# facebookresearch/jepa

Measured on AMD Instinct MI355X. Metric: V-JEPA pretrain clips/sec (fwd+bwd+EMA), higher is better.
Workload: dtype bf16; 1 GPU; V-JEPA pretrain step ViT-L/16 16x224x224, B=24/GPU, 2 multiblock masks (vitl16.yaml); global_batch=24, per_gpu_batch=24, parallelism=dp1, hw_queues=4

## Files before the change

### jepa_amd/csrc/common.hpp

```cpp
#pragma once
#include <hip/hip_runtime.h>
#include <stdint.h>
#include <stdio.h>

typedef uint16_t bf16_t;

typedef __attribute__((ext_vector_type(8))) __bf16 bf16x8_t;
typedef __attribute__((ext_vector_type(4))) float f32x4_t;
typedef __attribute__((ext_vector_type(4))) uint32_t u32x4_t;
typedef __attribute__((ext_vector_type(2))) uint32_t u32x2_t;

#define VJ_WAVE 64

__device__ __forceinline__ float bf2f(bf16_t v) { return __uint_as_float(((uint32_t)v) << 16); }

__device__ __forceinline__ bf16_t f2bf(float f) {
  uint32_t u = __float_as_uint(f);
  if ((u & 0x7fffffffu) > 0x7f800000u) return (bf16_t)((u >> 16) | 0x40u);
  u += 0x7fffu + ((u >> 16) & 1u);
  return (bf16_t)(u >> 16);
}
__device__ __forceinline__ uint32_t pack_bf2(float lo, float hi) {
  typedef __bf16 bf2_t __attribute__((ext_vector_type(2)));
  bf2_t v = {(__bf16)lo, (__bf16)hi};
  return __builtin_bit_cast(uint32_t, v);
}
__device__ __forceinline__ uint32_t pack_bf2_opaque(float lo, float hi) {
  uint32_t w = pack_bf2(lo, hi);
  asm("" : "+v"(w));
  return w;
}
__device__ __forceinline__ float bf_lo(uint32_t w) { return __uint_as_float(w << 16); }
__device__ __forceinline__ float bf_hi(uint32_t w) { return __uint_as_float(w & 0xffff0000u); }

__device__ __forceinline__ float wave_sum(float v) {
#pragma unroll
  for (int o = 32; o > 0; o >>= 1) v += __shfl_xor(v, o, 64);
  return v;
}
__device__ __forceinline__ float row16_sum(float v) {
  v += __int_as_float(__builtin_amdgcn_update_dpp(0, __float_as_int(v), 0x128, 0xf, 0xf, false));
  v += __int_as_float(__builtin_amdgcn_update_dpp(0, __float_as_int(v), 0x124, 0xf, 0xf, false));
  v += __int_as_float(__builtin_amdgcn_update_dpp(0, __float_as_int(v), 0x122, 0xf, 0xf, false));
  v += __int_as_float(__builtin_amdgcn_update_dpp(0, __float_as_int(v), 0x121, 0xf, 0xf, false));
  return v;
}
template <int N>
__device__ __forceinline__ void block4_stage(float (*red)[4], const float (&v)[N]) {
  float w[N];
#pragma unroll
  for (int k = 0; k < N; k++) w[k] = wave_sum(v[k]);
  if ((threadIdx.x & 63) == 0) {
#pragma unroll
    for (int k = 0; k < N; k++) red[k][threadIdx.x >> 6] = w[k];
  }
  __syncthreads();
}
__device__ __forceinline__ float block4_total(const float* red) { return red[0] + red[1] + red[2] + red[3]; }
__device__ __forceinline__ float wave_max(float v) {
#pragma unroll
  for (int o = 32; o > 0; o >>= 1) v = fmaxf(v, __shfl_xor(v, o, 64));
  return v;
}

typedef float f32x2_t __attribute__((ext_vector_type(2)));
__device__ __forceinline__ float twice_relu(float x) {
  float s;
  asm("v_add_f32 %0, %1, |%1|" : "=v"(s) : "v"(x));
  return s;
}
__device__ __forceinline__ f32x2_t half_erfc2_lp(f32x2_t x, f32x2_t& a) {
  a = (f32x2_t){__builtin_amdgcn_fmed3f(__builtin_fabsf(x[0]), 0.0f, 5.0f), __builtin_amdgcn_fmed3f(__builtin_fabsf(x[1]), 0.0f, 5.0f)};
  const f32x2_t c6 = {2.945814386e-05f, 2.945814386e-05f}, c5 = {-7.087827263e-04f, -7.087827263e-04f},
                 c4 = {7.746013931e-03f, 7.746013931e-03f}, c3 = {-5.260629358e-02f, -5.260629358e-02f},
                 c2 = {-4.596254594e-01f, -4.596254594e-01f}, c1 = {-1.150867238e+00f, -1.150867238e+00f},
                 c0 = {-1.000017643e+00f, -1.000017643e+00f};
  f32x2_t p = __builtin_elementwise_fma(c6, a, c5);
  p = __builtin_elementwise_fma(p, a, c4);
  p = __builtin_elementwise_fma(p, a, c3);
  p = __builtin_elementwise_fma(p, a, c2);
  p = __builtin_elementwise_fma(p, a, c1);
  p = __builtin_elementwise_fma(p, a, c0);
  return (f32x2_t){__builtin_amdgcn_exp2f(p[0]), __builtin_amdgcn_exp2f(p[1])};
}
__device__ __forceinline__ f32x2_t gelu2_lp(f32x2_t x) {
  f32x2_t a;
  const f32x2_t q = half_erfc2_lp(x, a);
  const f32x2_t s = {twice_relu(x[0]), twice_relu(x[1])};
  const f32x2_t half = {0.5f, 0.5f};
  return __builtin_elementwise_fma(s, half, -(a * q));
}
__device__ __forceinline__ void gelu_dgelu2_lp(f32x2_t x, f32x2_t& y, f32x2_t& d) {
  f32x2_t a;
  const f32x2_t q = half_erfc2_lp(x, a);
  const f32x2_t s = {twice_relu(x[0]), twice_relu(x[1])};
  const f32x2_t half = {0.5f, 0.5f};
  y = __builtin_elementwise_fma(s, half, -(a * q));
  const f32x2_t c = {-0.72134752044448170f, -0.72134752044448170f};
  const f32x2_t e = (x * c) * x;
  const f32x2_t g = {__builtin_amdgcn_exp2f(e[0]), __builtin_amdgcn_exp2f(e[1])};
  const f32x2_t hq = half - q;
  const f32x2_t phi = half + (f32x2_t){copysignf(hq[0], x[0]), copysignf(hq[1], x[1])};
  const f32x2_t k = {0.3989422804014327f, 0.3989422804014327f};
  d = __builtin_elementwise_fma(x * k, g, phi);
}

__device__ __forceinline__ int xcd_logical(int bid, int nblk) {
  const int qx = nblk >> 3, rx = nblk & 7, xcd = bid & 7, pos = bid >> 3;
  return (xcd < rx ? xcd * (qx + 1) : rx * (qx + 1) + (xcd - rx) * qx) + pos;
}

#include <atomic>
#define VJ_MAX_DEVICES 64
inline int vj_device_slot() {
  int dev = 0;
  if (hipGetDevice(&dev) != hipSuccess || dev < 0) dev = 0;
  return dev % VJ_MAX_DEVICES;
}
struct VjPerDeviceOnce {
  std::atomic<unsigned long long> done{0};
  template <class F>
  void operator()(F&& f) {
    const unsigned long long bit = 1ull << vj_device_slot();
    if (!(done.load(std::memory_order_acquire) & bit)) {
      f();
      done.fetch_or(bit, std::memory_order_release);
    }
  }
};

extern "C" const char* vj_last_error(void);
void vj_set_error(const char* fmt, ...);

#define VJ_CHECK_ARG(cond, ...)            \
  do {                                     \
    if (!(cond)) {                         \
      vj_set_error(__VA_ARGS__);           \
      return -1;                           \
    }                                      \
  } while (0)

#define VJ_LAUNCH_CHECK(name)                                              \
  do {                                                                     \
    hipError_t _e = hipGetLastError();                                     \
    if (_e != hipSuccess) {                                                \
      vj_set_error("%s: launch failed: %s", name, hipGetErrorString(_e)); \
      return (int)_e;                                                      \
    }                                                                      \
  } while (0)

__host__ __device__ static inline int64_t cdiv64(int64_t a, int64_t b) { return (a + b - 1) / b; }

static inline int rows_grid(int64_t rows, int64_t cap_blocks = 256 * 16) {
  int64_t g = cdiv64(rows, 4);
  if (g > cap_blocks) g = cap_blocks;
  if (g < 1) g = 1;
  return (int)g;
}
static inline int flat_grid(int64_t total, int64_t cap_blocks) {
  int64_t g = cdiv64(total, 256);
  if (g > cap_blocks) g = cap_blocks;
  return (int)g;
}
__device__ __forceinline__ int wave_lane() { return threadIdx.x & 63; }
__device__ __forceinline__ int64_t wave_row() { return (int64_t)blockIdx.x * 4 + (threadIdx.x >> 6); }
__device__ __forceinline__ int64_t wave_row_step() { return (int64_t)gridDim.x * 4; }

__device__ __forceinline__ void unpack8(const u32x4_t& w, float* v) {
#pragma unroll
  for (int i = 0; i < 4; i++) {
    v[2 * i] = bf_lo(w[i]);
    v[2 * i + 1] = bf_hi(w[i]);
  }
}
__device__ __forceinline__ void load8(const bf16_t* p, float* v) { unpack8(*(const u32x4_t*)p, v); }
__device__ __forceinline__ void store8(bf16_t* p, const float* v) {
  u32x4_t w;
#pragma unroll
  for (int i = 0; i < 4; i++) w[i] = pack_bf2(v[2 * i], v[2 * i + 1]);
  *(u32x4_t*)p = w;
}
__device__ __forceinline__ u32x2_t pack4_bf16(float a, float b, float c, float d) {
  u32x2_t w;
  w[0] = pack_bf2(a, b);
  w[1] = pack_bf2(c, d);
  return w;
}
__device__ __forceinline__ u32x4_t pack8_bf16(float4 lo, float4 hi) {
  u32x4_t o;
  o[0] = pack_bf2(lo.x, lo.y);
  o[1] = pack_bf2(lo.z, lo.w);
  o[2] = pack_bf2(hi.x, hi.y);
  o[3] = pack_bf2(hi.z, hi.w);
  return o;
}
__device__ __forceinline__ u32x4_t add_pos8(u32x4_t v, const float* pos) {
  const float4 p0 = *(const float4*)pos;
  const float4 p1 = *(const float4*)(pos + 4);
  v[0] = pack_bf2(bf_lo(v[0]) + p0.x, bf_hi(v[0]) + p0.y);
  v[1] = pack_bf2(bf_lo(v[1]) + p0.z, bf_hi(v[1]) + p0.w);
  v[2] = pack_bf2(bf_lo(v[2]) + p1.x, bf_hi(v[2]) + p1.y);
  v[3] = pack_bf2(bf_lo(v[3]) + p1.z, bf_hi(v[3]) + p1.w);
  return v;
}
```

### jepa_amd/csrc/layernorm.hip

```cpp
#include "common.hpp"
#include "options.hpp"
#include "internal.hpp"

#define LN_MAX_CHUNKS 4

static int ln_check_D(const char* who, int64_t D, bool rule = false) {
  VJ_CHECK_ARG(D % 8 == 0 && D <= 512 * LN_MAX_CHUNKS, rule ? "%s: D=%ld unsupported (need D%%8==0, D<=%d)" : "%s: D=%ld unsupported", who,
               (long)D, 512 * LN_MAX_CHUNKS);
  return 0;
}
static inline int ln_grid(int64_t rows) { return rows_grid(rows, 256 * 8); }

template <bool LOAD>
__device__ __forceinline__ float ln_row_mean(const bf16_t* xp, float (&v)[LN_MAX_CHUNKS][8], int lane, int D, float invD) {
  float s = 0.f;
#pragma unroll
  for (int i = 0; i < LN_MAX_CHUNKS; i++) {
    const int c = lane * 8 + i * 512;
    if (c < D) {
      if constexpr (LOAD) load8(xp + c, v[i]);
#pragma unroll
      for (int j = 0; j < 8; j++) s += v[i][j];
    }
  }
  return wave_sum(s) * invD;
}
__device__ __forceinline__ float ln_row_rstd(const float (&v)[LN_MAX_CHUNKS][8], float mean, int lane, int D, float invD, float eps) {
  float q = 0.f;
#pragma unroll
  for (int i = 0; i < LN_MAX_CHUNKS; i++) {
    if (lane * 8 + i * 512 < D) {
#pragma unroll
      for (int j = 0; j < 8; j++) {
        const float d = v[i][j] - mean;
        q += d * d;
      }
    }
  }
  return rsqrtf(wave_sum(q) * invD + eps);
}

__global__ __launch_bounds__(256) void layernorm_fwd_kernel(const bf16_t* __restrict__ x,
                                                            const float* __restrict__ gamma,
                                                            const float* __restrict__ beta, bf16_t* __restrict__ y,
                                                            float* __restrict__ mean_out, float* __restrict__ rstd_out,
                                                            int64_t rows, int D, float eps) {
  __shared__ __attribute__((aligned(16))) float4 gbs[LN_MAX_CHUNKS][4][64];
  const int lane = threadIdx.x & 63;
  for (int q = threadIdx.x; q < LN_MAX_CHUNKS * 64; q += 256) {
    const int i = q >> 6, l = q & 63, c = l * 8 + i * 512;
    if (c < D) {
      gbs[i][0][l] = *(const float4*)(gamma + c);
      gbs[i][1][l] = *(const float4*)(gamma + c + 4);
      gbs[i][2][l] = *(const float4*)(beta + c);
      gbs[i][3][l] = *(const float4*)(beta + c + 4);
    }
  }
  __syncthreads();
  const int64_t wave = (int64_t)blockIdx.x * 4 + (threadIdx.x >> 6);
  const int64_t nw = (int64_t)gridDim.x * 4;
  const float invD = 1.0f / (float)D;
  for (int64_t r = wave; r < rows; r += nw) {
    const bf16_t* xp = x + r * D;
    float v[LN_MAX_CHUNKS][8];
    const float mean = ln_row_mean<true>(xp, v, lane, D, invD);
    const float rstd = ln_row_rstd(v, mean, lane, D, invD, eps);
    bf16_t* yp = y + r * D;
#pragma unroll
    for (int i = 0; i < LN_MAX_CHUNKS; i++) {
      const int c = lane * 8 + i * 512;
      if (c < D) {
        const float4 g0 = gbs[i][0][lane], g1 = gbs[i][1][lane], b0 = gbs[i][2][lane], b1 = gbs[i][3][lane];
        const float gm[8] = {g0.x, g0.y, g0.z, g0.w, g1.x, g1.y, g1.z, g1.w};
        const float bt[8] = {b0.x, b0.y, b0.z, b0.w, b1.x, b1.y, b1.z, b1.w};
        float o[8];
#pragma unroll
        for (int j = 0; j < 8; j++) o[j] = (v[i][j] - mean) * rstd * gm[j] + bt[j];
        store8(yp + c, o);
      }
    }
    if (lane == 0 && mean_out) {
      mean_out[r] = mean;
      rstd_out[r] = rstd;
    }
  }
}

extern "C" int vj_layernorm_fwd(const void* x_bf16, const float* gamma, const float* beta, void* y_bf16, float* mean,
                                float* rstd, int64_t rows, int64_t D, float eps, hipStream_t stream) {
  if (ln_check_D("vj_layernorm_fwd", D, true)) return -1;
  VJ_CHECK_ARG((mean == nullptr) == (rstd == nullptr), "vj_layernorm_fwd: mean and rstd must both be given or both null");
  if (rows == 0) return 0;
  hipLaunchKernelGGL(layernorm_fwd_kernel, dim3(ln_grid(rows)), dim3(256), 0, stream, (const bf16_t*)x_bf16, gamma,
                     beta, (bf16_t*)y_bf16, mean, rstd, rows, (int)D, eps);
  VJ_LAUNCH_CHECK("vj_layernorm_fwd");
  return 0;
}

__global__ __launch_bounds__(256) void ln_rowstats_kernel(const bf16_t* __restrict__ x, float* __restrict__ rs, int64_t rows, int D,
                                                          float eps) {
  const int lane = threadIdx.x & 63;
  const int64_t wave = (int64_t)blockIdx.x * 4 + (threadIdx.x >> 6);
  const int64_t nw = (int64_t)gridDim.x * 4;
  const float invD = 1.0f / (float)D;
  for (int64_t r = wave; r < rows; r += nw) {
    const bf16_t* xp = x + r * D;
    float v[LN_MAX_CHUNKS][8];
    const float mean = ln_row_mean<true>(xp, v, lane, D, invD);
    const float rstd = ln_row_rstd(v, mean, lane, D, invD, eps);
    if (lane == 0) *(float2*)(rs + 2 * r) = make_float2(rstd, -mean * rstd);
  }
}

extern "C" int vj_ln_rowstats(const void* x_bf16, float* rowstats, int64_t rows, int64_t D, float eps, hipStream_t stream) {
  if (ln_check_D("vj_ln_rowstats", D, true)) return -1;
  VJ_CHECK_ARG(rowstats != nullptr && ((uintptr_t)rowstats % 8 == 0), "vj_ln_rowstats: rowstats null or misaligned");
  if (rows == 0) return 0;
  hipLaunchKernelGGL(ln_rowstats_kernel, dim3(ln_grid(rows)), dim3(256), 0, stream, (const bf16_t*)x_bf16, rowstats, rows, (int)D, eps);
  VJ_LAUNCH_CHECK("vj_ln_rowstats");
  return 0;
}

__global__ __launch_bounds__(256) void ln_fold_weights_kernel(const float* __restrict__ W, const float* __restrict__ b,
                                                              const float* __restrict__ gamma, const float* __restrict__ beta,
                                                              bf16_t* __restrict__ Wf, float* __restrict__ cvec, float* __restrict__ bf,
                                                              int64_t N, int K) {
  const int lane = threadIdx.x & 63;
  const int64_t n = (int64_t)blockIdx.x * 4 + (threadIdx.x >> 6);
  if (n >= N) return;
  const float* wp = W + n * K;
  bf16_t* op = Wf + n * K;
  float sc = 0.f, sb = 0.f;
  for (int k = lane * 4; k < K; k += 256) {
    const float4 w = *(const float4*)(wp + k);
    const float4 g = *(const float4*)(gamma + k);
    const float4 be = *(const float4*)(beta + k);
    u32x2_t o;
    o[0] = pack_bf2(w.x * g.x, w.y * g.y);
    o[1] = pack_bf2(w.z * g.z, w.w * g.w);
    *(u32x2_t*)(op + k) = o;
    sc += (bf_lo(o[0]) + bf_hi(o[0])) + (bf_lo(o[1]) + bf_hi(o[1]));
    sb += (w.x * be.x + w.y * be.y) + (w.z * be.z + w.w * be.w);
  }
  sc = wave_sum(sc);
  sb = wave_sum(sb);
  if (lane == 0) {
    cvec[n] = sc;
    bf[n] = (b ? b[n] : 0.f) + sb;
  }
}

extern "C" int vj_ln_fold_weights(const float* W, const float* b, const float* gamma, const float* beta, void* Wf_bf16, float* cvec,
                                  float* bf, int64_t N, int64_t K, hipStream_t stream) {
  VJ_CHECK_ARG(W != nullptr && gamma != nullptr && beta != nullptr && Wf_bf16 != nullptr && cvec != nullptr && bf != nullptr,
               "vj_ln_fold_weights: null pointer");
  VJ_CHECK_ARG(K % 4 == 0 && K > 0 && N >= 0 && K < (1 << 30), "vj_ln_fold_weights: K=%ld must be a positive multiple of 4", (long)K);
  VJ_CHECK_ARG((((uintptr_t)W | (uintptr_t)gamma | (uintptr_t)beta) % 16 == 0) && ((uintptr_t)Wf_bf16 % 8 == 0),
               "vj_ln_fold_weights: W / gamma / beta must be 16-byte aligned, Wf 8-byte aligned");
  if (N == 0) return 0;
  hipLaunchKernelGGL(ln_fold_weights_kernel, dim3((unsigned)cdiv64(N, 4)), dim3(256), 0, stream, W, b, gamma, beta, (bf16_t*)Wf_bf16,
                     cvec, bf, N, (int)K);
  VJ_LAUNCH_CHECK("vj_ln_fold_weights");
  return 0;
}

#define LN_BWD_MAX_BLOCKS 1024
template <int NCH, bool CS>
__global__ __launch_bounds__(256) void layernorm_bwd_kernel(const bf16_t* __restrict__ dy, const bf16_t* __restrict__ x,
                                                            const float* __restrict__ gamma,
                                                            const float* __restrict__ mean_in,
                                                            const float* __restrict__ rstd_in,
                                                            const bf16_t* __restrict__ dres, bf16_t* __restrict__ dx,
                                                            float* __restrict__ part, int64_t rows, int D) {
  constexpr int NSEG = CS ? 3 : 2;
  __shared__ float red[4][512 * NSEG];
  const int lane = threadIdx.x & 63, wv = threadIdx.x >> 6;
  const float invD = 1.0f / (float)D;
  float ag[NCH][8], ab[NCH][8], gam[NCH][8], as[CS ? NCH : 1][8];
#pragma unroll
  for (int i = 0; i < NCH; i++) {
    const int c = lane * 8 + i * 512;
#pragma unroll
    for (int j = 0; j < 8; j++) {
      ag[i][j] = ab[i][j] = 0.f;
      if constexpr (CS) as[i][j] = 0.f;
      gam[i][j] = (c < D) ? gamma[c + j] : 0.f;
    }
  }
  const int64_t rows_per = cdiv64(rows, gridDim.x);
  const int64_t rbeg = (int64_t)blockIdx.x * rows_per;
  const int64_t rend = (rbeg + rows_per < rows) ? rbeg + rows_per : rows;
  u32x4_t nx[NCH], nd[NCH], nr[NCH];
  float nmean = 0.f, nrstd = 0.f;
  auto request = [&](int64_t r) __attribute__((always_inline)) {
#pragma unroll
    for (int i = 0; i < NCH; i++) {
      const int c = lane * 8 + i * 512;
      if (c < D) {
        nx[i] = *(const u32x4_t*)(x + r * D + c);
        nd[i] = *(const u32x4_t*)(dy + r * D + c);
        if (dres) nr[i] = *(const u32x4_t*)(dres + r * D + c);
      }
    }
    nmean = mean_in[r];
    nrstd = rstd_in[r];
  };
#pragma unroll
  for (int i = 0; i < NCH; i++) nx[i] = nd[i] = nr[i] = (u32x4_t){0u, 0u, 0u, 0u};
  if (rbeg + wv < rend) request(rbeg + wv);
  for (int64_t r = rbeg + wv; r < rend; r += 4) {
    u32x4_t cx[NCH], cd[NCH], cr[NCH];
#pragma unroll
    for (int i = 0; i < NCH; i++) {
      cx[i] = nx[i];
      cd[i] = nd[i];
      cr[i] = nr[i];
    }
    const float mean = nmean, rstd = nrstd;
    if (r + 4 < rend) request(r + 4);
    float s1 = 0.f, s2 = 0.f;
#pragma unroll
    for (int i = 0; i < NCH; i++) {
      const int c = lane * 8 + i * 512;
      if (c < D) {
        float xv[8], dv[8];
        unpack8(cx[i], xv);
        unpack8(cd[i], dv);
#pragma unroll
        for (int j = 0; j < 8; j++) {
          const float xh = __fmul_rn(__fsub_rn(xv[j], mean), rstd);
          const float g = __fmul_rn(dv[j], gam[i][j]);
          s1 += g;
          s2 += g * xh;
          ag[i][j] += dv[j] * xh;
          ab[i][j] += dv[j];
        }
      }
    }
    const float c1 = wave_sum(s1) * invD, c2 = wave_sum(s2) * invD;
#pragma unroll
    for (int i = 0; i < NCH; i++) {
      const int c = lane * 8 + i * 512;
      if (c < D) {
        float o[8], xv[8], dv[8];
        unpack8(cx[i], xv);
        unpack8(cd[i], dv);
        if (dres) {
          unpack8(cr[i], o);
        } else {
#pragma unroll
          for (int j = 0; j < 8; j++) o[j] = 0.f;
        }
#pragma unroll
        for (int j = 0; j < 8; j++) {
          const float xh = __fmul_rn(__fsub_rn(xv[j], mean), rstd);
          const float g = __fmul_rn(dv[j], gam[i][j]);
          o[j] += rstd * (g - c1 - xh * c2);
        }
        if constexpr (CS) {
#pragma unroll
          for (int j = 0; j < 8; j++) as[i][j] += o[j];
        }
        store8(dx + r * D + c, o);
      }
    }
  }
  float* pg = part + (int64_t)blockIdx.x * NSEG * D;
#pragma unroll
  for (int i = 0; i < NCH; i++) {
    if (i * 512 < D) {
      __syncthreads();
#pragma unroll
      for (int j = 0; j < 8; j++) {
        red[wv][lane * 8 + j] = ag[i][j];
        red[wv][512 + lane * 8 + j] = ab[i][j];
        if constexpr (CS) red[wv][1024 + lane * 8 + j] = as[i][j];
      }
      __syncthreads();
      for (int q = threadIdx.x; q < 512 * NSEG; q += 256) {
        const int col = (q & 511) + i * 512;
        if (col < D) {
          const float s = red[0][q] + red[1][q] + red[2][q] + red[3][q];
          pg[(q >> 9) * D + col] = s;
        }
      }
    }
  }
}

extern "C" int64_t vj_layernorm_bwd_ws_bytes(int64_t D) { return (int64_t)LN_BWD_MAX_BLOCKS * 3 * D * 4; }

int vj_layernorm_bwd_partials(const void* dy_bf16, const void* x_bf16, const float* gamma, const float* mean, const float* rstd,
                              const void* dres_bf16, void* dx_bf16, bool cs, int64_t rows, int64_t D, void* ws,
                              int64_t ws_bytes, int64_t* nb_out, hipStream_t stream) {
  if (ln_check_D("vj_layernorm_bwd", D)) return -1;
  VJ_CHECK_ARG(ws_bytes >= vj_layernorm_bwd_ws_bytes(D), "vj_layernorm_bwd: workspace too small");
  *nb_out = 0;
  if (rows == 0) return 0;
  int64_t nb = cdiv64(rows, 16);
  if (nb > LN_BWD_MAX_BLOCKS) nb = LN_BWD_MAX_BLOCKS;
  if (nb < 1) nb = 1;
#define VJ_LNB(NCHV, CSV)                                                                                               \
  hipLaunchKernelGGL((layernorm_bwd_kernel<NCHV, CSV>), dim3((unsigned)nb), dim3(256), 0, stream, (const bf16_t*)dy_bf16, \
                     (const bf16_t*)x_bf16, gamma, mean, rstd, (const bf16_t*)dres_bf16, (bf16_t*)dx_bf16, (float*)ws,   \
                     rows, (int)D)
  if (cs) {
    if (D <= 512) VJ_LNB(1, true);
    else if (D <= 1024) VJ_LNB(2, true);
    else if (D <= 1536) VJ_LNB(3, true);
    else VJ_LNB(4, true);
  } else {
    if (D <= 512) VJ_LNB(1, false);
    else if (D <= 1024) VJ_LNB(2, false);
    else if (D <= 1536) VJ_LNB(3, false);
    else VJ_LNB(4, false);
  }
#undef VJ_LNB
  VJ_LAUNCH_CHECK("vj_layernorm_bwd");
  *nb_out = nb;
  return 0;
}

extern "C" int vj_layernorm_bwd_colsum(const void* dy_bf16, const void* x_bf16, const float* gamma, const float* mean,
                                       const float* rstd, const void* dres_bf16, void* dx_bf16, float* dgamma,
                                       float* dbeta, float* dxsum, float alpha, float beta_acc, int64_t rows, int64_t D,
                                       void* ws, int64_t ws_bytes, hipStream_t stream) {
  int64_t nb = 0;
  if (int rc = vj_layernorm_bwd_partials(dy_bf16, x_bf16, gamma, mean, rstd, dres_bf16, dx_bf16, dxsum != nullptr, rows, D, ws,
                                         ws_bytes, &nb, stream))
    return rc;
  if (nb == 0) return 0;
  float* outs[3] = {dgamma, dbeta, dxsum};
  return vj_reduce_partials_multi((const float*)ws, outs, dxsum != nullptr ? 3 : 2, nb, D, alpha, beta_acc, stream);
}

extern "C" int vj_layernorm_bwd(const void* dy_bf16, const void* x_bf16, const float* gamma, const float* mean,
                                const float* rstd, const void* dres_bf16, void* dx_bf16, float* dgamma, float* dbeta,
                                float alpha, float beta_acc, int64_t rows, int64_t D, void* ws, int64_t ws_bytes,
                                hipStream_t stream) {
  return vj_layernorm_bwd_colsum(dy_bf16, x_bf16, gamma, mean, rstd, dres_bf16, dx_bf16, dgamma, dbeta, nullptr, alpha,
                                 beta_acc, rows, D, ws, ws_bytes, stream);
}

__global__ __launch_bounds__(256) void target_rows_kernel(const bf16_t* __restrict__ x, const float* __restrict__ gamma,
                                                          const float* __restrict__ beta,
                                                          const int64_t* __restrict__ idx, float* __restrict__ h,
                                                          int64_t B, int64_t N, int64_t K, int D, float eps1,
                                                          float eps2) {
  const int lane = threadIdx.x & 63;
  const int64_t wave = (int64_t)blockIdx.x * 4 + (threadIdx.x >> 6);
  const int64_t nw = (int64_t)gridDim.x * 4;
  const float invD = 1.0f / (float)D;
  for (int64_t r = wave; r < B * K; r += nw) {
    const int64_t b = r / K;
    const bf16_t* xp = x + (b * N + idx[r]) * D;
    float v[LN_MAX_CHUNKS][8];
    float mean = ln_row_mean<true>(xp, v, lane, D, invD);
    float rstd = ln_row_rstd(v, mean, lane, D, invD, eps1);
#pragma unroll
    for (int i = 0; i < LN_MAX_CHUNKS; i++) {
      const int c = lane * 8 + i * 512;
      if (c < D) {
#pragma unroll
        for (int j = 0; j < 8; j++) v[i][j] = (v[i][j] - mean) * rstd * gamma[c + j] + beta[c + j];
      }
    }
    mean = ln_row_mean<false>(nullptr, v, lane, D, invD);
    rstd = ln_row_rstd(v, mean, lane, D, invD, eps2);
    float* hp = h + r * D;
#pragma unroll
    for (int i = 0; i < LN_MAX_CHUNKS; i++) {
      const int c = lane * 8 + i * 512;
      if (c < D) {
        float4 o0, o1;
        o0.x = (v[i][0] - mean) * rstd;
        o0.y = (v[i][1] - mean) * rstd;
        o0.z = (v[i][2] - mean) * rstd;
        o0.w = (v[i][3] - mean) * rstd;
        o1.x = (v[i][4] - mean) * rstd;
        o1.y = (v[i][5] - mean) * rstd;
        o1.z = (v[i][6] - mean) * rstd;
        o1.w = (v[i][7] - mean) * rstd;
        *(float4*)(hp + c) = o0;
        *(float4*)(hp + c + 4) = o1;
      }
    }
  }
}

extern "C" int vj_target_rows(const void* x_bf16, const float* gamma, const float* beta, const int64_t* idx,
                              float* h, int64_t B, int64_t N, int64_t K, int64_t D, float eps_norm, float eps_ln,
                              hipStream_t stream) {
  if (ln_check_D("vj_target_rows", D)) return -1;
  if (B * K == 0) return 0;
  hipLaunchKernelGGL(target_rows_kernel, dim3(ln_grid(B * K)), dim3(256), 0, stream, (const bf16_t*)x_bf16, gamma,
                     beta, idx, h, B, N, K, (int)D, eps_norm, eps_ln);
  VJ_LAUNCH_CHECK("vj_target_rows");
  return 0;
}
```

Measured before the change: 337.1 clips/s.

## Prefetch layernorm rows via buffer loads and specialize kernels by chunk count

The layernorm forward, rowstats and target-row kernels are rewritten around a shared row walker. It issues buffer loads for the next row before computing the current one, so memory latency overlaps the reductions. Each kernel is now templated on the chunk count chosen from D, which removes the dead chunk work and registers the old LN_MAX_CHUNKS loop carried. Out-of-range rows and stores are masked by zero-size buffer resources rather than branches, and the target kernel now stages gamma and beta in shared memory. The cost is higher register pressure from the prefetch buffers and more complex code.

```diff
diff --git a/jepa_amd/csrc/common.hpp b/jepa_amd/csrc/common.hpp
--- a/jepa_amd/csrc/common.hpp
+++ b/jepa_amd/csrc/common.hpp
@@ -180,6 +180,34 @@
   for (int i = 0; i < 4; i++) w[i] = pack_bf2(v[2 * i], v[2 * i + 1]);
   *(u32x4_t*)p = w;
 }
+typedef __amdgpu_buffer_rsrc_t row_rsrc_t;
+__device__ __forceinline__ row_rsrc_t row_rsrc(const void* base, int bytes) {
+  return __builtin_amdgcn_make_buffer_rsrc(const_cast<void*>(base), 0, bytes, 0x00020000);
+}
+__device__ __forceinline__ u32x4_t row_load16(row_rsrc_t row, int byte_offset) {
+  return __builtin_amdgcn_raw_buffer_load_b128(row, byte_offset, 0, 0);
+}
+__device__ __forceinline__ void row_store16(row_rsrc_t row, int byte_offset, u32x4_t w) {
+  __builtin_amdgcn_raw_buffer_store_b128(w, row, byte_offset, 0, 0);
+}
+__device__ __forceinline__ void row_store4(row_rsrc_t row, int byte_offset, float f) {
+  __builtin_amdgcn_raw_buffer_store_b32(__float_as_uint(f), row, byte_offset, 0, 0);
+}
+__device__ __forceinline__ void row_store8(row_rsrc_t row, int col, const float* v) {
+  u32x4_t w;
+#pragma unroll
+  for (int i = 0; i < 4; i++) w[i] = pack_bf2(v[2 * i], v[2 * i + 1]);
+  row_store16(row, col * 2, w);
+}
+__device__ __forceinline__ void row_store8_f32(row_rsrc_t row, int col, const float* v) {
+#pragma unroll
+  for (int h = 0; h < 2; h++) {
+    u32x4_t w;
+#pragma unroll
+    for (int i = 0; i < 4; i++) w[i] = __float_as_uint(v[4 * h + i]);
+    row_store16(row, (col + 4 * h) * 4, w);
+  }
+}
 __device__ __forceinline__ u32x2_t pack4_bf16(float a, float b, float c, float d) {
   u32x2_t w;
   w[0] = pack_bf2(a, b);
diff --git a/jepa_amd/csrc/layernorm.hip b/jepa_amd/csrc/layernorm.hip
--- a/jepa_amd/csrc/layernorm.hip
+++ b/jepa_amd/csrc/layernorm.hip
@@ -9,81 +9,164 @@
                (long)D, 512 * LN_MAX_CHUNKS);
   return 0;
 }
-static inline int ln_grid(int64_t rows) { return rows_grid(rows, 256 * 8); }
-
-template <bool LOAD>
-__device__ __forceinline__ float ln_row_mean(const bf16_t* xp, float (&v)[LN_MAX_CHUNKS][8], int lane, int D, float invD) {
+__device__ __forceinline__ float ln_rounded(float p) {
+  asm("" : "+v"(p));
+  return p;
+}
+
+template <int NCH>
+__device__ __forceinline__ float ln_row_mean(const float (&v)[NCH][8], int lane, int D, float invD) {
   float s = 0.f;
 #pragma unroll
-  for (int i = 0; i < LN_MAX_CHUNKS; i++) {
-    const int c = lane * 8 + i * 512;
-    if (c < D) {
-      if constexpr (LOAD) load8(xp + c, v[i]);
+  for (int i = 0; i < NCH; i++) {
+    if (lane * 8 + i * 512 < D) {
 #pragma unroll
       for (int j = 0; j < 8; j++) s += v[i][j];
     }
   }
-  return wave_sum(s) * invD;
-}
-__device__ __forceinline__ float ln_row_rstd(const float (&v)[LN_MAX_CHUNKS][8], float mean, int lane, int D, float invD, float eps) {
+  return ln_rounded(wave_sum(s) * invD);
+}
+template <int NCH>
+__device__ __forceinline__ float ln_row_rstd(const float (&v)[NCH][8], float mean, int lane, int D, float invD, float eps) {
   float q = 0.f;
 #pragma unroll
-  for (int i = 0; i < LN_MAX_CHUNKS; i++) {
+  for (int i = 0; i < NCH; i++) {
     if (lane * 8 + i * 512 < D) {
 #pragma unroll
       for (int j = 0; j < 8; j++) {
         const float d = v[i][j] - mean;
-        q += d * d;
-      }
-    }
-  }
-  return rsqrtf(wave_sum(q) * invD + eps);
-}
-
-__global__ __launch_bounds__(256) void layernorm_fwd_kernel(const bf16_t* __restrict__ x,
-                                                            const float* __restrict__ gamma,
-                                                            const float* __restrict__ beta, bf16_t* __restrict__ y,
-                                                            float* __restrict__ mean_out, float* __restrict__ rstd_out,
-                                                            int64_t rows, int D, float eps) {
-  __shared__ __attribute__((aligned(16))) float4 gbs[LN_MAX_CHUNKS][4][64];
-  const int lane = threadIdx.x & 63;
-  for (int q = threadIdx.x; q < LN_MAX_CHUNKS * 64; q += 256) {
+        q += ln_rounded(d * d);
+      }
+    }
+  }
+  return rsqrtf(__fmaf_rn(wave_sum(q), invD, eps));
+}
+
+#ifndef LN_FWD_MAX_BLOCKS
+#define LN_FWD_MAX_BLOCKS 2048
+#endif
+#define LN_ROWSTATS_MAX_BLOCKS 2048
+#ifndef LN_FWD_AHEAD
+#define LN_FWD_AHEAD 1
+#endif
+static inline int ln_fwd_grid(int64_t rows) {
+  const int64_t per_wave = cdiv64(rows, 4 * (int64_t)LN_FWD_MAX_BLOCKS);
+  return (int)cdiv64(rows, 4 * per_wave);
+}
+
+struct LnDenseRows {
+  const bf16_t* x;
+  int D;
+  __device__ __forceinline__ int64_t key(int64_t) const { return 0; }
+  __device__ __forceinline__ const bf16_t* row(int64_t r, int64_t) const { return x + r * D; }
+};
+struct LnGatheredRows {
+  const bf16_t* x;
+  const int64_t* idx;
+  int64_t N, K;
+  int D;
+  __device__ __forceinline__ int64_t key(int64_t r) const { return idx[r]; }
+  __device__ __forceinline__ const bf16_t* row(int64_t r, int64_t key) const { return x + ((r / K) * N + key) * D; }
+};
+
+template <int NCH, typename Rows, typename Staging, typename Body>
+__device__ __forceinline__ void ln_walk_rows(const Rows& src, int64_t rows, int D, Staging&& staging, Body&& body) {
+  constexpr int A = LN_FWD_AHEAD;
+  const int lane = wave_lane();
+  const int64_t nw = wave_row_step();
+  int64_t r = (int64_t)blockIdx.x * 4 + __builtin_amdgcn_readfirstlane((int)(threadIdx.x >> 6));
+  u32x4_t nx[A][NCH];
+  auto request = [&](int a, int64_t rr, int64_t key) __attribute__((always_inline)) {
+    const bool live = rr < rows;
+    const row_rsrc_t row = row_rsrc(live ? src.row(rr, key) : src.x, live ? D * 2 : 0);
+#pragma unroll
+    for (int i = 0; i < NCH; i++) nx[a][i] = row_load16(row, (lane * 8 + i * 512) * 2);
+  };
+  int64_t key[A + 1];
+#pragma unroll
+  for (int a = 0; a <= A; a++) key[a] = (r + a * nw < rows) ? src.key(r + a * nw) : 0;
+#pragma unroll
+  for (int a = 0; a < A; a++) request(a, r + a * nw, key[a]);
+  staging();
+  auto trip = [&]() __attribute__((always_inline)) {
+#pragma unroll
+    for (int a = 0; a < A; a++) {
+      const int64_t ra = r + a * nw;
+      float v[NCH][8];
+#pragma unroll
+      for (int i = 0; i < NCH; i++) unpack8(nx[a][i], v[i]);
+      __builtin_amdgcn_sched_barrier(0);
+      request(a, ra + A * nw, key[A]);
+      if (ra + (A + 1) * nw < rows) key[A] = src.key(ra + (A + 1) * nw);
+      body(ra, ra < rows, v);
+    }
+    r += A * nw;
+  };
+  if (r < rows) {
+    trip();
+    while (r < rows) trip();
+  }
+}
+
+template <int NCH>
+using ln_affine_t = float4[NCH][4][64];
+template <int NCH>
+__device__ __forceinline__ void ln_stage_affine(ln_affine_t<NCH>& gbs, const float* gamma, const float* beta, int D) {
+  for (int q = threadIdx.x; q < NCH * 64; q += 256) {
     const int i = q >> 6, l = q & 63, c = l * 8 + i * 512;
     if (c < D) {
       gbs[i][0][l] = *(const float4*)(gamma + c);
       gbs[i][1][l] = *(const float4*)(gamma + c + 4);
       gbs[i][2][l] = *(const float4*)(beta + c);
       gbs[i][3][l] = *(const float4*)(beta + c + 4);
+    } else {
+      gbs[i][0][l] = gbs[i][1][l] = gbs[i][2][l] = gbs[i][3][l] = make_float4(0.f, 0.f, 0.f, 0.f);
     }
   }
   __syncthreads();
-  const int64_t wave = (int64_t)blockIdx.x * 4 + (threadIdx.x >> 6);
-  const int64_t nw = (int64_t)gridDim.x * 4;
+}
+template <int NCH>
+__device__ __forceinline__ void ln_affine8(const ln_affine_t<NCH>& gbs, int i, int lane, const float* v, float mean, float rstd, float* o) {
+  const float4 g0 = gbs[i][0][lane], g1 = gbs[i][1][lane], b0 = gbs[i][2][lane], b1 = gbs[i][3][lane];
+  const float gm[8] = {g0.x, g0.y, g0.z, g0.w, g1.x, g1.y, g1.z, g1.w};
+  const float bt[8] = {b0.x, b0.y, b0.z, b0.w, b1.x, b1.y, b1.z, b1.w};
+#pragma unroll
+  for (int j = 0; j < 8; j++) o[j] = __fmaf_rn((v[j] - mean) * rstd, gm[j], bt[j]);
+}
+
+#define VJ_LN_FWD_LAUNCH(KERNEL, workgroups, ...)                                                                       \
+  do {                                                                                                                  \
+    const dim3 grid_(workgroups), block_(256);                                                                          \
+    if (D <= 512) hipLaunchKernelGGL((KERNEL<1>), grid_, block_, 0, stream, __VA_ARGS__);                               \
+    else if (D <= 1024) hipLaunchKernelGGL((KERNEL<2>), grid_, block_, 0, stream, __VA_ARGS__);                         \
+    else if (D <= 1536) hipLaunchKernelGGL((KERNEL<3>), grid_, block_, 0, stream, __VA_ARGS__);                         \
+    else hipLaunchKernelGGL((KERNEL<4>), grid_, block_, 0, stream, __VA_ARGS__);                                        \
+  } while (0)
+
+template <int NCH>
+__global__ __launch_bounds__(256) void layernorm_fwd_kernel(const bf16_t* __restrict__ x,
+                                                            const float* __restrict__ gamma,
+                                                            const float* __restrict__ beta, bf16_t* __restrict__ y,
+                                                            float* __restrict__ mean_out, float* __restrict__ rstd_out,
+                                                            int64_t rows, int D, float eps) {
+  __shared__ __attribute__((aligned(16))) ln_affine_t<NCH> gbs;
+  const int lane = wave_lane();
   const float invD = 1.0f / (float)D;
-  for (int64_t r = wave; r < rows; r += nw) {
-    const bf16_t* xp = x + r * D;
-    float v[LN_MAX_CHUNKS][8];
-    const float mean = ln_row_mean<true>(xp, v, lane, D, invD);
-    const float rstd = ln_row_rstd(v, mean, lane, D, invD, eps);
-    bf16_t* yp = y + r * D;
-#pragma unroll
-    for (int i = 0; i < LN_MAX_CHUNKS; i++) {
-      const int c = lane * 8 + i * 512;
-      if (c < D) {
-        const float4 g0 = gbs[i][0][lane], g1 = gbs[i][1][lane], b0 = gbs[i][2][lane], b1 = gbs[i][3][lane];
-        const float gm[8] = {g0.x, g0.y, g0.z, g0.w, g1.x, g1.y, g1.z, g1.w};
-        const float bt[8] = {b0.x, b0.y, b0.z, b0.w, b1.x, b1.y, b1.z, b1.w};
-        float o[8];
-#pragma unroll
-        for (int j = 0; j < 8; j++) o[j] = (v[i][j] - mean) * rstd * gm[j] + bt[j];
-        store8(yp + c, o);
-      }
-    }
-    if (lane == 0 && mean_out) {
-      mean_out[r] = mean;
-      rstd_out[r] = rstd;
-    }
-  }
+  ln_walk_rows<NCH>(
+      LnDenseRows{x, D}, rows, D, [&]() __attribute__((always_inline)) { ln_stage_affine<NCH>(gbs, gamma, beta, D); },
+      [&](int64_t r, bool live, const float (&v)[NCH][8]) __attribute__((always_inline)) {
+        const float mean = ln_row_mean<NCH>(v, lane, D, invD);
+        const float rstd = ln_row_rstd<NCH>(v, mean, lane, D, invD, eps);
+        const row_rsrc_t yrow = row_rsrc(y + r * D, live ? D * 2 : 0);
+#pragma unroll
+        for (int i = 0; i < NCH; i++) {
+          float o[8];
+          ln_affine8<NCH>(gbs, i, lane, v[i], mean, rstd, o);
+          row_store8(yrow, lane * 8 + i * 512, o);
+        }
+        row_store4(row_rsrc(mean_out + r, live && mean_out ? 4 : 0), lane * 4, mean);
+        row_store4(row_rsrc(rstd_out + r, live && mean_out ? 4 : 0), lane * 4, rstd);
+      });
 }
 
 extern "C" int vj_layernorm_fwd(const void* x_bf16, const float* gamma, const float* beta, void* y_bf16, float* mean,
@@ -91,32 +174,32 @@
   if (ln_check_D("vj_layernorm_fwd", D, true)) return -1;
   VJ_CHECK_ARG((mean == nullptr) == (rstd == nullptr), "vj_layernorm_fwd: mean and rstd must both be given or both null");
   if (rows == 0) return 0;
-  hipLaunchKernelGGL(layernorm_fwd_kernel, dim3(ln_grid(rows)), dim3(256), 0, stream, (const bf16_t*)x_bf16, gamma,
-                     beta, (bf16_t*)y_bf16, mean, rstd, rows, (int)D, eps);
+  VJ_LN_FWD_LAUNCH(layernorm_fwd_kernel, ln_fwd_grid(rows), (const bf16_t*)x_bf16, gamma, beta, (bf16_t*)y_bf16, mean, rstd, rows, (int)D, eps);
   VJ_LAUNCH_CHECK("vj_layernorm_fwd");
   return 0;
 }
 
+template <int NCH>
 __global__ __launch_bounds__(256) void ln_rowstats_kernel(const bf16_t* __restrict__ x, float* __restrict__ rs, int64_t rows, int D,
                                                           float eps) {
-  const int lane = threadIdx.x & 63;
-  const int64_t wave = (int64_t)blockIdx.x * 4 + (threadIdx.x >> 6);
-  const int64_t nw = (int64_t)gridDim.x * 4;
+  const int lane = wave_lane();
   const float invD = 1.0f / (float)D;
-  for (int64_t r = wave; r < rows; r += nw) {
-    const bf16_t* xp = x + r * D;
-    float v[LN_MAX_CHUNKS][8];
-    const float mean = ln_row_mean<true>(xp, v, lane, D, invD);
-    const float rstd = ln_row_rstd(v, mean, lane, D, invD, eps);
-    if (lane == 0) *(float2*)(rs + 2 * r) = make_float2(rstd, -mean * rstd);
-  }
+  ln_walk_rows<NCH>(
+      LnDenseRows{x, D}, rows, D, []() {},
+      [&](int64_t r, bool live, const float (&v)[NCH][8]) __attribute__((always_inline)) {
+        const float mean = ln_row_mean<NCH>(v, lane, D, invD);
+        const float rstd = ln_row_rstd<NCH>(v, mean, lane, D, invD, eps);
+        const row_rsrc_t out = row_rsrc(rs + 2 * r, live ? 8 : 0);
+        row_store4(out, lane * 8, rstd);
+        row_store4(out, lane * 8 + 4, -mean * rstd);
+      });
 }
 
 extern "C" int vj_ln_rowstats(const void* x_bf16, float* rowstats, int64_t rows, int64_t D, float eps, hipStream_t stream) {
   if (ln_check_D("vj_ln_rowstats", D, true)) return -1;
   VJ_CHECK_ARG(rowstats != nullptr && ((uintptr_t)rowstats % 8 == 0), "vj_ln_rowstats: rowstats null or misaligned");
   if (rows == 0) return 0;
-  hipLaunchKernelGGL(ln_rowstats_kernel, dim3(ln_grid(rows)), dim3(256), 0, stream, (const bf16_t*)x_bf16, rowstats, rows, (int)D, eps);
+  VJ_LN_FWD_LAUNCH(ln_rowstats_kernel, rows_grid(rows, LN_ROWSTATS_MAX_BLOCKS), (const bf16_t*)x_bf16, rowstats, rows, (int)D, eps);
   VJ_LAUNCH_CHECK("vj_ln_rowstats");
   return 0;
 }
@@ -342,50 +425,34 @@
                                  beta_acc, rows, D, ws, ws_bytes, stream);
 }
 
+template <int NCH>
 __global__ __launch_bounds__(256) void target_rows_kernel(const bf16_t* __restrict__ x, const float* __restrict__ gamma,
                                                           const float* __restrict__ beta,
                                                           const int64_t* __restrict__ idx, float* __restrict__ h,
                                                           int64_t B, int64_t N, int64_t K, int D, float eps1,
                                                           float eps2) {
-  const int lane = threadIdx.x & 63;
-  const int64_t wave = (int64_t)blockIdx.x * 4 + (threadIdx.x >> 6);
-  const int64_t nw = (int64_t)gridDim.x * 4;
+  __shared__ __attribute__((aligned(16))) ln_affine_t<NCH> gbs;
+  const int lane = wave_lane();
   const float invD = 1.0f / (float)D;
-  for (int64_t r = wave; r < B * K; r += nw) {
-    const int64_t b = r / K;
-    const bf16_t* xp = x + (b * N + idx[r]) * D;
-    float v[LN_MAX_CHUNKS][8];
-    float mean = ln_row_mean<true>(xp, v, lane, D, invD);
-    float rstd = ln_row_rstd(v, mean, lane, D, invD, eps1);
-#pragma unroll
-    for (int i = 0; i < LN_MAX_CHUNKS; i++) {
-      const int c = lane * 8 + i * 512;
-      if (c < D) {
-#pragma unroll
-        for (int j = 0; j < 8; j++) v[i][j] = (v[i][j] - mean) * rstd * gamma[c + j] + beta[c + j];
-      }
-    }
-    mean = ln_row_mean<false>(nullptr, v, lane, D, invD);
-    rstd = ln_row_rstd(v, mean, lane, D, invD, eps2);
-    float* hp = h + r * D;
-#pragma unroll
-    for (int i = 0; i < LN_MAX_CHUNKS; i++) {
-      const int c = lane * 8 + i * 512;
-      if (c < D) {
-        float4 o0, o1;
-        o0.x = (v[i][0] - mean) * rstd;
-        o0.y = (v[i][1] - mean) * rstd;
-        o0.z = (v[i][2] - mean) * rstd;
-        o0.w = (v[i][3] - mean) * rstd;
-        o1.x = (v[i][4] - mean) * rstd;
-        o1.y = (v[i][5] - mean) * rstd;
-        o1.z = (v[i][6] - mean) * rstd;
-        o1.w = (v[i][7] - mean) * rstd;
-        *(float4*)(hp + c) = o0;
-        *(float4*)(hp + c + 4) = o1;
-      }
-    }
-  }
+  ln_walk_rows<NCH>(
+      LnGatheredRows{x, idx, N, K, D}, B * K, D, [&]() __attribute__((always_inline)) { ln_stage_affine<NCH>(gbs, gamma, beta, D); },
+      [&](int64_t r, bool live, const float (&raw)[NCH][8]) __attribute__((always_inline)) {
+        float v[NCH][8];
+        float mean = ln_row_mean<NCH>(raw, lane, D, invD);
+        float rstd = ln_row_rstd<NCH>(raw, mean, lane, D, invD, eps1);
+#pragma unroll
+        for (int i = 0; i < NCH; i++) ln_affine8<NCH>(gbs, i, lane, raw[i], mean, rstd, v[i]);
+        mean = ln_row_mean<NCH>(v, lane, D, invD);
+        rstd = ln_row_rstd<NCH>(v, mean, lane, D, invD, eps2);
+        const row_rsrc_t hrow = row_rsrc(h + r * D, live ? D * 4 : 0);
+#pragma unroll
+        for (int i = 0; i < NCH; i++) {
+          float o[8];
+#pragma unroll
+          for (int j = 0; j < 8; j++) o[j] = (v[i][j] - mean) * rstd;
+          row_store8_f32(hrow, lane * 8 + i * 512, o);
+        }
+      });
 }
 
 extern "C" int vj_target_rows(const void* x_bf16, const float* gamma, const float* beta, const int64_t* idx,
@@ -393,8 +460,7 @@
                               hipStream_t stream) {
   if (ln_check_D("vj_target_rows", D)) return -1;
   if (B * K == 0) return 0;
-  hipLaunchKernelGGL(target_rows_kernel, dim3(ln_grid(B * K)), dim3(256), 0, stream, (const bf16_t*)x_bf16, gamma,
-                     beta, idx, h, B, N, K, (int)D, eps_norm, eps_ln);
+  VJ_LN_FWD_LAUNCH(target_rows_kernel, ln_fwd_grid(B * K), (const bf16_t*)x_bf16, gamma, beta, idx, h, B, N, K, (int)D, eps_norm, eps_ln);
   VJ_LAUNCH_CHECK("vj_target_rows");
   return 0;
 }
```

Measured after the change: 336.9 clips/s, median of 2. No clear change (-0.1%).
